# ishine/StyleTTS-ZS

Measured on AMD Instinct MI355X. Metric: synthesized audio-sec/sec (whole job) + p50 utterance latency, 3-s ref -> 5-s target, higher is better.
Workload: dtype bf16; 1 GPU; configs[2]: batch 64/GPU, 5-s targets, 2-step distilled style diffusion, CFG 5; global_batch=64, seq_len=200, parallelism=dp1 (utterance shards), spec=v0, graph=True, branch_streams=False, streams=2, schedule=pipe, stagger=0

## Files before the change

### include/stzs.h

```cpp
#ifndef STZS_H
#define STZS_H

#include <stddef.h>
#include <stdint.h>

#ifdef __cplusplus
extern "C" {
#endif

#define STZS_OK 0
#define STZS_EINVAL (-1)
#define STZS_ESHAPE (-2)
#define STZS_EDTYPE (-3)
#define STZS_EHIP (-4)

enum { STZS_F32 = 0, STZS_BF16 = 1, STZS_I32 = 2, STZS_F8 = 3  };
enum { STZS_ACT_NONE = 0, STZS_ACT_LEAKY = 1, STZS_ACT_SNAKE = 2, STZS_ACT_GELU = 3, STZS_ACT_SILU = 4 };
enum { STZS_PRO_NONE = 0, STZS_PRO_ADAIN = 1 };
#define STZS_CONV_A_DMA 8

int stzs_init(int device);
const char* stzs_strerror(int code);
int stzs_version(void);

// ... 42 lines not shown
#define STZS_CONV_UPS_NOISE 4096
#define STZS_CONV_MRFV_NARROW 8192
#define STZS_CONV_W_FRAG32X3 16384
#define STZS_CONV_MRFV_T128 32768
#define STZS_CONV_RING 65536
#define STZS_CONV_SK_TICKET 131072
size_t stzs_conv_rows_workspace(int64_t rows, int32_t Co, int32_t kgroups);
int stzs_conv1d(const stzs_conv_args* a, void* stream);
int stzs_conv1d_group(const stzs_conv_args* a, int n, void* stream);

typedef struct stzs_stats_args {
    const void* x;
    float* mean;
    float* rstd;
    void* partial;
    int64_t ld, bs, stat_bs;
    int32_t B, T, C, dtype;
    float eps, pad_f;
} stzs_stats_args;
size_t stzs_chan_stats_workspace(int B, int T, int C);
int stzs_chan_stats(const stzs_stats_args* a, void* stream);
int stzs_chan_stats_partial(const stzs_stats_args* a, void* stream);
int stzs_chan_stats_final(const stzs_stats_args* a, int chunk_rows, void* stream);
int stzs_chan_stats_final_group(const stzs_stats_args* a, int n, int chunk_rows, void* stream);

typedef struct stzs_rowln_args {
    const void* x;
    void* y;
    const float* G;
    const float* Bt;
    int64_t ldx, ldy, gs, bs;
    int32_t R, C, gdiv, in_dtype, out_dtype, act;
    float gadd, eps, slope, pad_f;
    float* y_scale;
} stzs_rowln_args;
int stzs_row_layernorm(const stzs_rowln_args* a, void* stream);
int stzs_ln_linear(const stzs_conv_args* a, const stzs_rowln_args* ln, void* stream);

typedef struct stzs_quant_args {
    const void* x;
    void* y;
    float* scale;
    int64_t ldx, ldy;
    int32_t R, C;
} stzs_quant_args;
int stzs_quant_rows(const stzs_quant_args* a, void* stream);
// ... 281 lines not shown
```

### styletts-zs_amd/csrc/norm.hip

```cpp
#include "common.hpp"
#include "rowln.hpp"

namespace {

constexpr int STAT_ROWS = 256;
constexpr int STAT_CG = 32;

template <typename T>
__global__ __launch_bounds__(256) void chan_stats_partial(const stzs_stats_args a, int nchunk) {
    __shared__ float red[8][STAT_CG * 8][2];
    const int tid = threadIdx.x, tx = tid & 31, ty = tid >> 5;
    const int chunk = blockIdx.x, b = blockIdx.y;
    const int cv = blockIdx.z * STAT_CG + tx;
    const int c = cv * 8;
    float s[8], q[8];
#pragma unroll
    for (int j = 0; j < 8; ++j) s[j] = q[j] = 0.f;
    const int r0 = chunk * STAT_ROWS, r1 = min(a.T, r0 + STAT_ROWS);
    const T* X = reinterpret_cast<const T*>(a.x) + (long)b * a.bs;
    if (c < a.C) {
        int r = r0 + ty;
        for (; r + 24 < r1; r += 32) {
            float v[4][8];
#pragma unroll
// ... 62 lines not shown
            s += (double)v.x;
            q += (double)v.y;
        }
    }
    red[g][cl][0] = s;
    red[g][cl][1] = q;
    __syncthreads();
    if (tid < FIN_CH && c < a.C) {
        s = q = 0.0;
#pragma unroll
        for (int y = 0; y < 8; ++y) {
            s += red[y][tid][0];
            q += red[y][tid][1];
        }
        float mu, rs;
        stat_finish(s, q, a.T, a.eps, mu, rs);
        a.mean[(long)b * a.stat_bs + c] = mu;
        a.rstd[(long)b * a.stat_bs + c] = rs;
    }
}

__global__ __launch_bounds__(256) void chan_stats_final(const stzs_stats_args a, int nchunk) {
    stats_final_body(a, nchunk, blockIdx.x, blockIdx.y);
}

struct StatsGroup {
    stzs_stats_args a[3];
    int nchunk[3];
};
__global__ __launch_bounds__(256) void chan_stats_final_group(const StatsGroup g) {
    const int z = blockIdx.z;
    const stzs_stats_args& a = z == 0 ? g.a[0] : (z == 1 ? g.a[1] : g.a[2]);
    if ((int)blockIdx.x >= a.B || (int)blockIdx.y * FIN_CH >= a.C) return;
    stats_final_body(a, z == 0 ? g.nchunk[0] : (z == 1 ? g.nchunk[1] : g.nchunk[2]), blockIdx.x, blockIdx.y);
}


template <typename TI, typename TO>
__global__ __launch_bounds__(256) void row_ln(const stzs_rowln_args a) {
    const long r = (long)blockIdx.x * 4 + (threadIdx.x >> 6);
    if (r >= a.R) return;
    stzs_ln::row_ln_one<TI, TO>(a, r, threadIdx.x & 63);
}

__global__ __launch_bounds__(256) void quant_rows(const stzs_quant_args a) {
    constexpr int MAXV = 4;
// ... 45 lines not shown
    if (rc != STZS_OK) return rc;
    STZS_LAUNCH_CHECK();
    return STZS_OK;
}

extern "C" int stzs_chan_stats(const stzs_stats_args* a, void* stream) {
    if (!a || !a->x || !a->mean || !a->rstd || !a->partial) return STZS_EINVAL;
    hipStream_t s = reinterpret_cast<hipStream_t>(stream);
    int nchunk = 0;
    const int rc = chan_stats_pass1(a, s, &nchunk);
    if (rc != STZS_OK) return rc;
    STZS_LAUNCH_CHECK();
    hipLaunchKernelGGL(chan_stats_final, dim3(a->B, (a->C + FIN_CH - 1) / FIN_CH), dim3(256), 0, s, *a, nchunk);
    STZS_LAUNCH_CHECK();
    return STZS_OK;
}

extern "C" int stzs_chan_stats_final(const stzs_stats_args* a, int chunk_rows, void* stream) {
    if (!a || !a->mean || !a->rstd || !a->partial) return STZS_EINVAL;
    if (a->B <= 0 || a->T <= 0 || a->C <= 0 || chunk_rows <= 0) return STZS_ESHAPE;
    hipStream_t s = reinterpret_cast<hipStream_t>(stream);
    const int nchunk = (a->T + chunk_rows - 1) / chunk_rows;
    hipLaunchKernelGGL(chan_stats_final, dim3(a->B, (a->C + FIN_CH - 1) / FIN_CH), dim3(256), 0, s, *a, nchunk);
    STZS_LAUNCH_CHECK();
    return STZS_OK;
}

extern "C" int stzs_chan_stats_final_group(const stzs_stats_args* a, int n, int chunk_rows, void* stream) {
    if (!a || n < 1 || n > 3 || chunk_rows <= 0) return STZS_EINVAL;
    StatsGroup g = {};
    int gx = 0, gy = 0;
    for (int i = 0; i < n; ++i) {
        if (!a[i].mean || !a[i].rstd || !a[i].partial) return STZS_EINVAL;
        if (a[i].B <= 0 || a[i].T <= 0 || a[i].C <= 0) return STZS_ESHAPE;
        g.a[i] = a[i];
        g.nchunk[i] = (a[i].T + chunk_rows - 1) / chunk_rows;
        gx = a[i].B > gx ? a[i].B : gx;
        const int ny = (a[i].C + FIN_CH - 1) / FIN_CH;
        gy = ny > gy ? ny : gy;
    }
    hipLaunchKernelGGL(chan_stats_final_group, dim3(gx, gy, n), dim3(256), 0, reinterpret_cast<hipStream_t>(stream), g);
    STZS_LAUNCH_CHECK();
    return STZS_OK;
}

extern "C" int stzs_row_layernorm(const stzs_rowln_args* a, void* stream) {
// ... 37 lines not shown
```

### styletts-zs_amd/csrc/ups.hip

```cpp
#include "common.hpp"

namespace {

constexpr int NTH = 256;
#ifndef STZS_UPS_P
#define STZS_UPS_P 288
#endif
constexpr int P = STZS_UPS_P;
constexpr int rows_of(int bt) { return bt + 1; }
constexpr int tile_of(int bt) { return (rows_of(bt) * P + 15) & ~15; }
constexpr int RING = 4;

template <int NCH, bool HR, bool NZ, int BT = 128>
__global__ __launch_bounds__(NTH, NCH * tile_of(BT) <= 80 * 1024 ? 2 : 1) void ups_conv(const stzs_conv_args a, int ctw) {
    extern __shared__ __attribute__((aligned(16))) unsigned char smem[];
    constexpr int ROWS = rows_of(BT), TILE = tile_of(BT);
    constexpr int SB = (ROWS + 15) / 16;
    constexpr int MT = BT / 16;
    constexpr int NK = NCH * 8;
    constexpr int NKW = NK + (NZ ? 1 : 0);
    const int tid = threadIdx.x, lane = tid & 63, wave = tid >> 6;
    const int tpb = (a.T_out + BT - 1) / BT;
    const int nx = gridDim.x;
    const int lin = (a.flags & STZS_CONV_LINEAR_IDS) ? blockIdx.y * nx + blockIdx.x
                                                      : xcd_remap(blockIdx.y * nx + blockIdx.x, nx * gridDim.y);
    const int gy = lin / nx, bx = lin - gy * nx;
    const int bq = bx / tpb;
    const int q0 = (bx - bq * tpb) * BT;
    const int ncol = a.ups * a.Co;
    const int nct = (ncol + 127) / 128;
    const int ct0 = gy * ctw, ct1 = min(nct, ct0 + ctw);
    const int J = (ct1 - ct0) * NK;
    const bf16x8* Wf = reinterpret_cast<const bf16x8*>(a.w) + (long)ct0 * NKW * 512 + wave * 128 + lane;
    bf16x8 wf[RING][2];
// ... 24 lines not shown
#pragma unroll
        for (int i = 0; i < SB; ++i) {
            const int r = rsub + 16 * i;
            const int tin = q0 - 1 + r;
            const bool ok = c_ok && tin >= 0 && tin < a.T_in;
            const uint32_t w[4] = {raw[i].x, raw[i].y, raw[i].z, raw[i].w};
            uint32_t o[4];
#pragma unroll
            for (int p = 0; p < 4; ++p) {
                float y0 = __uint_as_float(w[p] << 16) + 0.f, y1 = __uint_as_float(w[p] & 0xFFFF0000u) + 0.f;
                if (lrelu) {
                    y0 = y0 >= 0.f ? y0 : y0 * slope;
                    y1 = y1 >= 0.f ? y1 : y1 * slope;
                }
                o[p] = ok ? pack2bf(y0, y1) : 0u;
            }
            if (r < ROWS) *reinterpret_cast<uint4*>(smem + cc * TILE + r * P + cv * 16) = make_uint4(o[0], o[1], o[2], o[3]);
        }
    }
    __syncthreads();
    const int g = lane >> 4, n = lane & 15;
    const int xoff0 = (lane & 15) * P + (lane >> 4) * 16;
    const int t_hi = a.T_final + a.refl - 1;
    const bf16_t* Rb = reinterpret_cast<const bf16_t*>(a.res) + (long)bq * a.bsr;
    bf16_t* Y = reinterpret_cast<bf16_t*>(a.y) + (long)bq * a.bsy;
    f32x4 acc[2][MT];
    bf16x8 xf[MT];
    for (int ct = ct0; ct < ct1; ++ct) {
        const int jb = (ct - ct0) * NK;
        const int col0 = ct * 128 + wave * 32 + g * 8;
        const int ph = col0 / a.Co, cof = col0 - ph * a.Co;
        const bool col_ok = col0 < ncol;
        const int cofc = col_ok ? cof : 0;
        uint4 rr[MT];
        int trow[MT];
#pragma unroll
        for (int mt = 0; mt < MT; ++mt) {
            const int q = q0 + mt * 16 + n;
            const int t = q * a.ups + ph - a.ups_pad + a.refl;
            trow[mt] = t;
            const int tc = t < 0 ? 0 : (t > t_hi ? t_hi : t);
            if constexpr (NZ) rr[mt] = *reinterpret_cast<const uint4*>(Rb + (long)tc * a.ldr + g * 8);
            else if constexpr (HR) rr[mt] = *reinterpret_cast<const uint4*>(Rb + (long)tc * a.ldr + cofc);
        }
        bf16x8 wn[2];
        if constexpr (NZ) {
// ... 27 lines not shown
            __builtin_amdgcn_sched_barrier(0);
        }
        if constexpr (NZ) {
#pragma unroll
            for (int mt = 0; mt < MT; ++mt) {
                const bf16x8 hf = __builtin_bit_cast(bf16x8, rr[mt]);
                acc[0][mt] = __builtin_amdgcn_mfma_f32_16x16x32_bf16(wn[0], hf, acc[0][mt], 0, 0, 0);
                acc[1][mt] = __builtin_amdgcn_mfma_f32_16x16x32_bf16(wn[1], hf, acc[1][mt], 0, 0, 0);
            }
        }
        if (a.flags & 4) continue;
        float corr[8] = {0.f, 0.f, 0.f, 0.f, 0.f, 0.f, 0.f, 0.f};
        if constexpr (NZ) {
            if (a.refl && q0 == 0 && n == 0 && trow[0] == 2 && col_ok) {
#pragma unroll 1
                for (int j = 0; j < 32; ++j) {
                    const float d = bf2f(Rb[j]) - bf2f(Rb[2 * a.ldr + j]);
#pragma unroll
                    for (int i = 0; i < 8; ++i) corr[i] = fmaf(a.gate[(long)(cof + i) * 32 + j], d, corr[i]);
                }
            }
        }
#pragma unroll
        for (int mt = 0; mt < MT; ++mt) {
            const int q = q0 + mt * 16 + n;
            const int t = trow[mt];
            const int tp = t - a.refl;
            const bool ok = col_ok && q < a.T_out && tp >= 0 && tp < a.T_final;
            float v[8];
#pragma unroll
            for (int nt = 0; nt < 2; ++nt)
#pragma unroll
                for (int r = 0; r < 4; ++r) v[nt * 4 + r] = acc[nt][mt][r] + bias[nt * 4 + r];
            float w0[8];
#pragma unroll
            for (int i = 0; i < 8; ++i) w0[i] = v[i];
            if constexpr (HR) {
                float f[8];
                unpack8(rr[mt], f);
#pragma unroll
                for (int i = 0; i < 8; ++i) v[i] += f[i];
            }
#pragma unroll
            for (int i = 0; i < 8; ++i) v[i] *= a.alpha;
            if (ok) *reinterpret_cast<uint4*>(Y + (long)t * a.ldy + cof) = pack8(v);
            if (a.refl && ok && t == 2) {
                if constexpr (NZ) {
#pragma unroll
                    for (int i = 0; i < 8; ++i) w0[i] += corr[i];
                } else if constexpr (HR) {
                    float f[8];
                    load8(Rb + cof, f);
#pragma unroll
                    for (int i = 0; i < 8; ++i) w0[i] += f[i];
                }
#pragma unroll
                for (int i = 0; i < 8; ++i) w0[i] *= a.alpha;
                *reinterpret_cast<uint4*>(Y + cof) = pack8(w0);
            }
        }
    }
}

}

__attribute__((visibility("hidden"))) int stzs_ups_conv_launch(const stzs_conv_args& a, hipStream_t s) {
    const bool nz = (a.flags & STZS_CONV_UPS_NOISE) != 0;
    if (nz && (!a.res || !a.gate || a.Co % 128 || a.refl < 0 || a.refl > 1 || a.ldr < 32 || a.ldr % 8 || a.bsr % 8 ||
               (a.refl && a.T_final + a.refl < 3)))
        return STZS_EINVAL;
    if (a.ks != 2 || a.pad != 1 || a.dil != 1 || a.stride != 1 || a.cic != 128 || a.ci_pad % 128 || a.Co % 32 ||
        a.T_out != a.T_in + 1 || a.in_dtype != STZS_BF16 || a.out_dtype != STZS_BF16 || a.pro_mode != STZS_PRO_NONE ||
        (a.pro_act != STZS_ACT_LEAKY && a.pro_act != STZS_ACT_NONE) || a.pro_cscale != 1.f || (a.gate && !nz) || a.acc_in ||
        a.stat_part || a.epi_act != STZS_ACT_NONE || a.ldy % 8 || a.bsy % 8 ||
        (a.res && (a.ldr % 8 || a.bsr % 8 || a.res_tdiv != 1)) || a.co_pad < a.ups * a.Co)
        return STZS_ESHAPE;
    const int nch = a.ci_pad / 128;
    const int nct = (a.ups * a.Co + 127) / 128;
    static const int bt_env = [] {
        const char* e = getenv("STZS_UPS_BT");
        return e ? atoi(e) : 0;
    }();
    const int BT = bt_env == 64 || bt_env == 128 ? bt_env : (nch > 2 ? 64 : 128);
    const int nqt = a.B * ((a.T_out + BT - 1) / BT);
    const int target = 4 * stzs_cu_count();
    int groups = 1;
    while (groups < nct && (long)nqt * groups < target) ++groups;
    const int ctw = (nct + groups - 1) / groups;
    groups = (nct + ctw - 1) / ctw;
    const size_t lds = (size_t)nch * (BT == 64 ? tile_of(64) : tile_of(128));
    void (*k)(stzs_conv_args, int) = nullptr;
    const bool R = a.res != nullptr;
#define STZS_UPS_PICK(N, B_)                                                                                    \
    k = nz ? ups_conv<N, false, true, B_> : R ? ups_conv<N, true, false, B_> : ups_conv<N, false, false, B_>;
    switch (nch * (BT == 64 ? -1 : 1)) {
        case 1: STZS_UPS_PICK(1, 128) break;
        case 2: STZS_UPS_PICK(2, 128) break;
// ... 15 lines not shown
```

### styletts-zs_amd/stzs/_lib.py

```python
from __future__ import annotations

import ctypes as C
import os

_HERE = os.path.dirname(os.path.abspath(__file__))
LIB_PATH = os.environ.get("STZS_LIB", os.path.join(_HERE, "libstzs_hip.so"))

F32, BF16, I32, F8 = 0, 1, 2, 3
OK, EINVAL, ESHAPE, EDTYPE, EHIP = 0, -1, -2, -3, -4
ACT_NONE, ACT_LEAKY, ACT_SNAKE, ACT_GELU, ACT_SILU = 0, 1, 2, 3, 4
PRO_NONE, PRO_ADAIN = 0, 1
CONV_STAT_ROWS = 64
CONV_W_LANE16 = 16
CONV_W_NARROW32 = 32
CONV_W_FRAG32 = 256
CONV_W_F32 = 64
CONV_W_X3 = 1024
CONV_LINEAR_IDS = 128
CONV_ROWS = 2048
CONV_UPS_NOISE = 4096
CONV_MRFV_NARROW = 8192
CONV_MRFV_T128 = 32768
CONV_RING = 65536
CONV_SK_TICKET = 131072
# ... 157 lines not shown
    d = Tensor()
    d.data = t.data_ptr()
    d.dtype = dtype if dtype is not None else {torch.float32: F32, torch.bfloat16: BF16, torch.int32: I32,
                                                torch.float8_e4m3fn: F8, torch.uint8: BF16}[t.dtype]
    d.ndim = t.dim()
    for k in range(t.dim()):
        d.shape[k] = t.shape[k]
        d.stride[k] = t.stride(k)
    return d


def params(ints=(), floats=()) -> Params:
    p = Params()
    for k, v in enumerate(ints):
        p.i[k] = int(v)
    for k, v in enumerate(floats):
        p.f[k] = float(v)
    return p


EXPORTS = ["stzs_init", "stzs_strerror", "stzs_version", "stzs_conv1d", "stzs_conv1d_group", "stzs_conv_splitk_workspace",
           "stzs_conv_rows_workspace",
           "stzs_chan_stats_workspace",
           "stzs_chan_stats", "stzs_chan_stats_partial", "stzs_chan_stats_final", "stzs_chan_stats_final_group", "stzs_row_layernorm", "stzs_ln_linear", "stzs_quant_rows", "stzs_attention", "stzs_lstm_workspace", "stzs_lstm", "stzs_lstm_pair",
           "stzs_lstm_state_reset", "stzs_predictor_prep",
           "stzs_durations", "stzs_alignment", "stzs_gather_rows", "stzs_adain_dwup", "stzs_f0n_down",
           "stzs_harmonic_source", "stzs_istft", "stzs_istft_stream", "stzs_istft_stream_span",
           "stzs_stft_frames", "stzs_log_mel", "stzs_stft_logmel", "stzs_pool_rows", "stzs_code_quantize",
           "stzs_dn_cond", "stzs_dn_cond_steps", "stzs_adaln_expand", "stzs_cfg_euler",
           "stzs_state_init", "stzs_mean_rows", "stzs_copy2d", "stzs_embed", "stzs_embed_f32", "stzs_dn_cond_steps_f32", "stzs_pack_conv_size", "stzs_pack_conv",
           "stzs_pack_lstm", "stzs_pack_lstm_x3"] + [f"stzs_{o}{sfx}" for o in GENERIC_OPS for sfx in ("", "_workspace")]

_lib = None


class StzsError(RuntimeError):
    pass


def load():
    global _lib
    if _lib is not None:
        return _lib
    if not os.path.exists(LIB_PATH):
        raise StzsError(f"libstzs_hip.so not found at {LIB_PATH}: run `python styletts-zs_amd/build.py` "
                        "(the product path has no CPU fallback)")
    L = C.CDLL(LIB_PATH)
    P = C.POINTER
    sig = {
        "stzs_init": ([i32], i32),
        "stzs_strerror": ([i32], C.c_char_p),
        "stzs_version": ([], i32),
        "stzs_conv1d": ([P(ConvArgs), vp], i32),
        "stzs_conv1d_group": ([P(ConvArgs), i32, vp], i32),
        "stzs_conv_splitk_workspace": ([i64, i32, i32], C.c_size_t),
        "stzs_conv_rows_workspace": ([i64, i32, i32], C.c_size_t),
        "stzs_chan_stats_workspace": ([i32, i32, i32], C.c_size_t),
        "stzs_chan_stats": ([P(StatsArgs), vp], i32),
        "stzs_chan_stats_partial": ([P(StatsArgs), vp], i32),
        "stzs_chan_stats_final": ([P(StatsArgs), i32, vp], i32),
        "stzs_chan_stats_final_group": ([P(StatsArgs), i32, i32, vp], i32),
        "stzs_row_layernorm": ([P(RowLNArgs), vp], i32),
        "stzs_ln_linear": ([P(ConvArgs), P(RowLNArgs), vp], i32),
        "stzs_quant_rows": ([P(QuantArgs), vp], i32),
        "stzs_attention": ([P(AttnArgs), vp], i32),
        "stzs_lstm_workspace": ([i32, i32, i32], C.c_size_t),
        "stzs_lstm": ([P(LstmArgs), vp], i32),
        "stzs_lstm_pair": ([P(LstmArgs), P(LstmArgs), vp], i32),
        "stzs_lstm_state_reset": ([vp, vp, vp], i32),
        "stzs_predictor_prep": ([P(PrPrepArgs), vp], i32),
        "stzs_durations": ([P(DurArgs), vp], i32),
        "stzs_alignment": ([P(AlignArgs), vp], i32),
        "stzs_gather_rows": ([P(GatherArgs), vp], i32),
        "stzs_adain_dwup": ([P(DwupArgs), vp], i32),
        "stzs_f0n_down": ([P(F0nArgs), vp], i32),
        "stzs_harmonic_source": ([P(SourceArgs), vp], i32),
        "stzs_istft": ([P(IstftArgs), vp], i32),
        "stzs_istft_stream": ([P(IstftStreamArgs), vp], i32),
        "stzs_istft_stream_span": ([i32, i32, i32, i32, i32, P(i64), P(i64)], i32),
        "stzs_stft_frames": ([P(FramesArgs), vp], i32),
        "stzs_log_mel": ([P(LogMelArgs), vp], i32),
        "stzs_stft_logmel": ([P(StftMelArgs), vp], i32),
        "stzs_pool_rows": ([P(PoolArgs), vp], i32),
# ... 36 lines not shown
```

### styletts-zs_amd/stzs/engine.py

```python
from __future__ import annotations

import ctypes as C
import math
import os
from dataclasses import dataclass
from functools import partial

import numpy as np
import torch

from . import _lib as L
from .spec import Spec
from .weights import ConvW, PackedModel

_DT = {torch.float32: L.F32, torch.bfloat16: L.BF16, torch.float8_e4m3fn: L.F8}
DN_SPLITK = {}
LATENCY_DN_SPLITK = dict(ff2=4)
DN_ROWS = {}
LATENCY_DN_ROWS = dict(inp=1, qkv=1, o=1, q=1, co=1, ff1=1, ff2=4, out=1)
TE_SPLITK = 0
LATENCY_TE_SPLITK = 4
BLK_SPLITK = 0
LATENCY_BLK_SPLITK = 16

# ... 34 lines not shown


def _on(v):
    return v != "0"


_KNOBS = (
    ("dur_overlap", "STZS_DUR_OVERLAP", "1", lambda v: bool(int(v))),
    ("dn_splitk", "STZS_DN_SPLITK", DN_SPLITK, _table),
    ("dn_rows", "STZS_DN_ROWS", DN_ROWS, _table),
    ("te_splitk", "STZS_TE_SPLITK", TE_SPLITK, int),
    ("blk_splitk", "STZS_BLK_SPLITK", BLK_SPLITK, int),
    ("defer_stats", "STZS_DEFER_STATS", lambda eng: "1" if eng.blk_splitk else "0", _on),
    ("mrf_trio", "STZS_MRF_TRIO", "1", _on),
    ("f0n_pair", "STZS_F0N_PAIR", "1", _on),
    ("kv_fuse", "STZS_KV_FUSE", "1", _on),
    ("small_rows", "STZS_SMALL_ROWS", "1", _on),
    ("ln_fuse", "STZS_LN_FUSE", "1", _on),
    ("rows16", "STZS_ROWS16", "1", _on),
    ("rows16_split", "STZS_ROWS16_SPLIT", "1", _on),
    ("rows16_maxk", "STZS_ROWS16_MAXK", "512", int),
    ("ups_noise_fused", "STZS_UPS_NOISE", "1", _on),
    ("noise_super", "STZS_NOISE_SUPER", "1", _on),
    ("mrfx", "STZS_MRFX", "1", _on),
    ("conv_flags", "STZS_CONV_FLAGS", "0", lambda v: int(v, 0)),
)


def _rup(x, m):
    return (x + m - 1) // m * m


@dataclass
class Act:
    t: torch.Tensor
    c0: int = 0
    C: int = -1

    def __post_init__(self):
        if self.C < 0:
            self.C = self.t.shape[-1] - self.c0

    @property
    def B(self):
        return self.t.shape[0]

# ... 28 lines not shown
    if steps == 1:
        return [spec.sigma_max, 0.0]
    if steps == 2:
        return [spec.sigma_max, 0.5, 0.0]
    lo, hi = spec.sigma_min ** (1 / spec.rho), spec.sigma_max ** (1 / spec.rho)
    return [(hi + i / (steps - 1) * (lo - hi)) ** spec.rho for i in range(steps)] + [0.0]


def edm_coeffs(spec: Spec, sigma: float):
    sd = spec.sigma_data
    return dict(c_in=1.0 / math.sqrt(sigma ** 2 + sd ** 2), c_skip=sd ** 2 / (sigma ** 2 + sd ** 2),
                c_out=sigma * sd / math.sqrt(sigma ** 2 + sd ** 2), c_noise=math.log(sigma) / 4.0)


def fourier_features(spec: Spec, c_noise: float) -> np.ndarray:
    half = spec.dn_fourier // 2
    f = np.exp(-math.log(10000.0) * np.arange(half) / half)
    arg = 1000.0 * c_noise * f
    return np.concatenate([np.cos(arg), np.sin(arg)]).astype(np.float32)


class _StatsRef:

    def __init__(self, eng, part, ld, nch, T, B, mean, rstd, chunk_rows):
        self.eng, self.part, self.ld, self.nch, self.T, self.B = eng, part, ld, nch, T, B
        self.mean, self.rstd, self.chunk_rows, self.done = mean, rstd, chunk_rows, False

    def final_args(self, s):
        s.mean, s.rstd, s.partial = self.mean.data_ptr(), self.rstd.data_ptr(), self.part.data_ptr()
        s.stat_bs, s.B, s.T, s.C, s.eps = self.ld, self.B, self.T, self.ld, 1e-5
        return s

    def finalize(self):
        if not self.done:
            self.eng._raw(self.eng.lib.stzs_chan_stats_final, "chan_stats_final",
                          C.byref(self.final_args(L.StatsArgs())), self.chunk_rows)
            self.done = True

    def mean_ptr(self):
        self.finalize()
        return self.mean.data_ptr()

    def rstd_ptr(self):
        self.finalize()
        return self.rstd.data_ptr()


class _StatPtr:

    def __init__(self, ref, which):
        self.ref, self.which = ref, which

    def data_ptr(self):
        return self.ref.mean_ptr() if self.which == 0 else self.ref.rstd_ptr()

    def tensor(self):
        self.ref.finalize()
        return self.ref.mean if self.which == 0 else self.ref.rstd

# ... 134 lines not shown
        if rows > 1 or splitk > 1:
            self._conv_splitk(a, cw, x, splitk, rows, collect, what)
        if pro_ref is not None:
            self._conv_stats_in(a, cw, pro_ref, pre_ln)
        st = self._conv_stats_out(a, cw, y, stats_key, collect) if stats_key is not None else None
        fn, args, fused = self._conv_entry(a, cw, x, res, res_tdiv, gate, pre_ln, st)
        if collect is not None:
            assert len(args) == 1 and pre_ln is None and post_ln is None and attn is None, what
            collect.append(a)
        else:
            if pre_ln is not None and not fused:
                self._call(self.lib.stzs_row_layernorm, pre_ln, what + ".ln", cost=_ln_cost(pre_ln))
            rec = {} if self.timer is None else dict(
                shape=(cw.ks, dil, a.T_out, cw.Co),
                cost=partial(_conv_cost, cw, x, y, a.T_out, res, acc_in, pre_ln if fused else None))
            self._call(fn, a, what, args=args, **rec)
        if post_ln is not None:
            self._call(self.lib.stzs_row_layernorm, post_ln, what + ".ln", cost=_ln_cost(post_ln))
        if attn is not None:
            self.attention(*attn)
        if st is None:
            return y
        slab, Cc, mean, rstd, defer, ntile = st
        ref = _StatsRef(self, slab, Cc, ntile, a.T_out, y.B, mean, rstd, L.CONV_STAT_ROWS)
        if not defer:
            ref.finalize()
            return y, (mean, rstd, Cc)
        return y, (_StatPtr(ref, 0), _StatPtr(ref, 1), Cc)

    def _conv_fill(self, cw, x, y, what, *, T_out, pad, dil, stride, pro, pro_act, pro_slope, pro_alpha, cscale, res,
                   res_tdiv, acc_in, alpha, beta, gate, gate_bs, epi_act, epi_slope, ups_pad, T_final, refl, x_scale):
        a = L.ConvArgs()
        a.x, a.w, a.y = x.ptr, self._t(cw.w).data_ptr(), y.ptr
        a.bias = self._t(cw.b).data_ptr() if cw.b is not None else None
        a.ldx, a.bsx, a.ldy, a.bsy = x.ld, x.bs, y.ld, y.bs
        T = x.T
        a.B, a.T_in, a.Ci, a.Co, a.ks, a.dil, a.stride, a.pad = x.B, T, cw.Ci, cw.Co, cw.ks, dil, stride, pad
        assert x.C == cw.Ci, (what, x.C, cw.Ci)
        if cw.ups:
            a.T_out = T + 1
            a.ups, a.ups_pad, a.T_final, a.refl = cw.ups, ups_pad, T_final, refl
            a.pad = 1
        else:
            a.T_out = T_out if T_out is not None else (T + 2 * pad - dil * (cw.ks - 1) - 1) // stride + 1
        a.ci_pad, a.co_pad, a.cic = cw.ci_pad, cw.co_pad, cw.cic
        a.in_dtype, a.out_dtype = x.dt, y.dt
        pro_ref = None
# ... 82 lines not shown
            splitk = min(splitk, 16, cw.ci_pad // cw.cic)
        if splitk > 1 and (a.flags & 8) and not cw.f8 and cw.wx3 is None and cw.w32 is None:
            nb = self.lib.stzs_conv_splitk_workspace(x.B * x.T, cw.co_pad, splitk)
            assert nb > 0, (what, splitk)
            a.splitk, a.splitk_ws = splitk, self._scratch("sk_ws", nb // 4).data_ptr()
            a.splitk_ctr = self._counters("sk_ctr", nb // (splitk * 32768)).data_ptr()
        elif splitk > 1 and _conv_generic(a.flags, cw):
            tiles = x.B * ((a.T_out + 127) // 128) * (cw.co_pad // 128)
            a.splitk = splitk
            gs = f".g{len(collect)}" if collect is not None else ""
            a.splitk_ws = self._scratch("csk_ws" + gs, tiles * splitk * 16384).data_ptr()
            a.splitk_ctr = self._counters("csk_ctr" + gs, tiles).data_ptr()

    def _conv_stats_in(self, a, cw, pro_ref, pre_ln):
        if _conv_generic(a.flags, cw) and pre_ln is None and pro_ref.nch <= 8:
            a.pro_part, a.pro_ld, a.pro_nch, a.pro_T, a.pro_eps = pro_ref.part.data_ptr(), pro_ref.ld, pro_ref.nch, \
                pro_ref.T, 1e-5
        else:
            a.pro_mean, a.pro_rstd = pro_ref.mean_ptr(), pro_ref.rstd_ptr()

    def _conv_stats_out(self, a, cw, y, stats_key, collect):
        Cc = _rup(cw.Co, 8)
        ntile = (a.T_out + L.CONV_STAT_ROWS - 1) // L.CONV_STAT_ROWS
        defer = collect is not None or (self.defer_stats and ntile <= 8)
        slab = self._scratch("stat_slab." + stats_key, y.B * ntile * Cc * 2, 1024) if defer else \
            self._scratch("stat_slab", y.B * ntile * Cc * 2)
        a.stat_part, a.stat_ld = slab.data_ptr(), Cc
        return (slab, Cc, self.buf(stats_key + ".m", (y.B, Cc), torch.float32),
                self.buf(stats_key + ".r", (y.B, Cc), torch.float32), defer, ntile)

    def _conv_entry(self, a, cw, x, res, res_tdiv, gate, pre_ln, st):
        if not (a.flags & L.CONV_ROWS):
            return self.lib.stzs_conv1d, (C.byref(a),), False
        nk = cw.ci_pad // 32
        if pre_ln is not None:
            fused = a.splitk <= 1 and res is None and gate is None and \
                st is None and pre_ln.C == cw.Ci == cw.ci_pad and nk in (4, 8, 16) and pre_ln.out_dtype == L.BF16 and \
                pre_ln.act == L.ACT_NONE and (pre_ln.x or 0) % 16 == 0 and pre_ln.ldx % 8 == 0 and \
                pre_ln.gdiv > 0 and pre_ln.R < (1 << 22) - 16 and \
                (not pre_ln.G or (pre_ln.gs % 8 == 0 and pre_ln.G % 32 == 0)) and \
                (not pre_ln.Bt or (pre_ln.bs % 8 == 0 and pre_ln.Bt % 32 == 0))
            if fused:
                return self.lib.stzs_ln_linear, (C.byref(a), C.byref(pre_ln)), True
        r16 = (pre_ln is None and self.rows16 and st is None and
               (res is None or res_tdiv == 1) and x.ptr % 16 == 0 and x.ld % 8 == 0 and x.bs % 8 == 0)
        r16_split = r16 and self.rows16_split and a.splitk in (2, 4) and nk % a.splitk == 0 and \
            nk // a.splitk in (4, 8, 16)
# ... 714 lines not shown
            sd = self._consts.get(skey)
            if sd is None:
                host = torch.as_tensor(np.asarray(seeds, dtype=np.uint32).view(np.int32).copy())
                sd = self._consts[skey] = host.to(self.device)
        pref = self.buf("gen.pref", (B, nh, T80), torch.float32)
        dt = self.dec_dt
        hb = self.buf("gen.har", (B, self._har_rows(Tf), _rup(S.har_ch, 32)), dt, zero=True)
        har = Act(hb[:, :Tf], 0, S.har_ch)
        a = L.SourceArgs()
        a.f0, a.seeds, a.merge_w, a.prefix, a.har = F0.data_ptr(), sd.data_ptr(), W.t(W.src_merge).data_ptr(), \
            pref.data_ptr(), har.ptr
        a.ldf, a.ldh, a.bsh = F0.stride(0), har.ld, har.bs
        a.B, a.T80, a.hop, a.n_fft, a.hop_s, a.nh = B, T80, S.hop, S.n_fft, S.istft_hop, nh
        a.sr, a.sine_amp, a.noise_std, a.voiced_thr = float(S.sr), S.sine_amp, S.noise_std, S.voiced_threshold
        a.har_dtype = har.dt
        self._call(self.lib.stzs_harmonic_source, a, "harmonic_source",
                   cost=(0, B * T80 * 4 * (1 + 2 * nh) + B * Tf * S.har_ch * har.t.element_size()))
        return har

    def _har_rows(self, Tf: int) -> int:
        s = math.prod(self.spec.up_rates[1:]) if len(self.spec.up_rates) > 1 else 1
        return _rup(Tf, s)

    def upsample(self, x: Act, har: Act, i: int) -> Act:
        S, W = self.spec, self.W
        B = x.B
        n_up = len(S.up_rates)
        r, k = S.up_rates[i], S.up_kernels[i]
        c = S.gen_ch[i]
        last = i == n_up - 1
        Tcur = x.T
        Tn = Tcur * r + (1 if last else 0)
        dt = self.dec_dt
        xu = self.act(f"gen.x{i}", B, Tn, c, dt)
        nzw = self.W.ups_nz[i] if (self.ups_noise_fused and i < len(self.W.ups_nz)) else None
        if nzw is not None and dt == torch.bfloat16 and har.ld >= 32:
            self.conv(nzw, x, xu, pro_act=L.ACT_LEAKY, pro_slope=0.1, ups_pad=(k - r) // 2, T_final=Tcur * r,
                      refl=1 if last else 0, res=Act(har.t, 0, har.ld), flags=L.CONV_UPS_NOISE,
                      gate=self._t(nzw.nz32).data_ptr(), what=f"ups{i}")
            return xu
        xsrc = self.act(f"gen.xsrc{i}", B, Tn, c, dt)
        sup = W.noise_sup[i] if (not last and i < len(W.noise_sup)) else None
        sf0 = int(np.prod(S.up_rates[i + 1:])) if not last else 1
        rows_alloc = har.bs // har.ld
        if (sup is not None and self.noise_super and har.dt == L.BF16 and har.bs % (sf0 * har.ld) == 0 and
                rows_alloc // sf0 >= Tn + 1 and sf0 * har.ld == sup.Ci and har.t.stride(1) == har.ld):
            hs = har.t.as_strided((B, rows_alloc // sf0, sf0 * har.ld), (har.bs, sf0 * har.ld, 1))
            self.conv(sup, Act(hs), xsrc, pad=1, T_out=Tn, what=f"noise_conv{i}")
        elif not last:
            self.conv(W.noise_conv[i], har.sl(0, S.har_ch), xsrc, stride=sf0, pad=(sf0 + 1) // 2, T_out=Tn,
                      what=f"noise_conv{i}")
        else:
            self.conv(W.noise_conv[i], har.sl(0, S.har_ch), xsrc, T_out=Tn, what=f"noise_conv{i}")
        self.conv(W.ups[i], x, xu, pro_act=L.ACT_LEAKY, pro_slope=0.1, ups_pad=(k - r) // 2, T_final=Tcur * r,
                  refl=1 if last else 0, res=xsrc, what=f"ups{i}")
        return xu

    def conv_post(self, x: Act) -> Act:
        S, W = self.spec, self.W
        post = self.act("gen.post", x.B, x.T, S.har_ch, torch.float32)
        self.conv(W.conv_post, x, Act(post.t, 0, S.har_ch), pad=3, pro_act=L.ACT_LEAKY, pro_slope=0.01,
                  what="conv_post")
        return post

    def istft(self, post: Act) -> torch.Tensor:
        S = self.spec
        B, Tcur = post.B, post.T
        Nout = (Tcur - 1) * S.istft_hop
        wav = self.buf("gen.wav", (B, Nout), torch.float32)
        a = L.IstftArgs()
        a.post, a.wav, a.ldp, a.bsp, a.bsw = post.ptr, wav.data_ptr(), post.ld, post.bs, Nout
        a.B, a.Tf, a.n_fft, a.hop_s = B, Tcur, S.n_fft, S.istft_hop
        self._call(self.lib.stzs_istft, a, "istft", cost=(0, B * Tcur * S.har_ch * 4 + B * Nout * 4))
        return wav

    def generator(self, x: Act, F0: torch.Tensor, seeds, gbd, trace=None, istft=True, har: Act = None):
        S, W = self.spec, self.W
        ng = W.dec_norm
        if har is None:
            har = self.sine_gen(F0, seeds)
        if trace is not None:
            trace["har"] = har
        for i in range(len(S.up_rates)):
            xu = self.upsample(x, har, i)
            if trace is not None:
                trace[f"mrf_in{i}"] = xu
            x = self.mrf(xu, i, gbd, ng)
            if trace is not None:
                trace[f"mrf_out{i}"] = x
        post = self.conv_post(x)
        if trace is not None:
            trace["post"] = post
        if not istft:
            return post
        return self.istft(post)

    def _istft_chunk(self, rows_ptr, ldp, bsp, B, f0, Fc, fin, wav, tails, i):
        S = self.spec
        n0, n1 = C.c_int64(), C.c_int64()
        halo = self.lib.stzs_istft_stream_span(f0, Fc, fin, S.n_fft, S.istft_hop, C.byref(n0), C.byref(n1))
        L.check(min(halo, 0), "istft_stream_span")
        assert halo <= 8
        a = L.IstftStreamArgs()
        a.post = rows_ptr
        a.tail_in = tails[i % 2].data_ptr() if f0 > 0 else None
        a.tail_out = tails[(i + 1) % 2].data_ptr() if not fin else None
        a.wav = wav.data_ptr() + n0.value * 4
        a.ldp, a.bsp, a.bsw, a.ldt = ldp, bsp, wav.shape[1], tails[0].shape[2]
        a.B, a.f0, a.Fc, a.final_chunk, a.n_fft, a.hop_s = B, f0, Fc, fin, S.n_fft, S.istft_hop
        self._call(self.lib.stzs_istft_stream, a, "istft_stream")
# ... 101 lines not shown
        self.launches += rc

    def _finalize_group(self, refs):
        arr = (L.StatsArgs * len(refs))()
        for s, r in zip(arr, refs):
            r.final_args(s)
        assert len({r.chunk_rows for r in refs}) == 1
        self._raw(self.lib.stzs_chan_stats_final_group, "chan_stats_final_group", arr, len(refs), refs[0].chunk_rows)
        for r in refs:
            r.done = True

    def _rb_c1(self, lw, x: Act, y: Act, st, gbd, ng, stats_key, collect=None):
        k, dil = lw["k"], lw["dil"]
        o1, c1 = ng.offsets[lw["n1"]]
        return self.conv(lw["c1"], x, y, pad=dil * (k - 1) // 2, dil=dil,
                         pro=(*st, gbd.data_ptr() + o1 * 4, ng.total, c1), pro_act=L.ACT_SNAKE, pro_alpha=lw["a1"],
                         stats_key=stats_key, collect=collect, what="rb.c1")[1]

    def _rb_c2(self, lw, x: Act, y: Act, st, res: Act, gbd, ng, **kw):
        o2, c2 = ng.offsets[lw["n2"]]
        return self.conv(lw["c2"], x, y, pad=(lw["k"] - 1) // 2, pro=(*st, gbd.data_ptr() + o2 * 4, ng.total, c2),
                         pro_act=L.ACT_SNAKE, pro_alpha=lw["a2"], res=res, what="rb.c2", **kw)

    def _mrf_trio(self, x: Act, i, gbd, ng):
        S, W = self.spec, self.W
        B, T, c = x.B, x.T, x.C
        dt = x.t.dtype
        nk = len(S.rb_kernels)
        xs = self.act(f"gen.xs{i}", B, T, c, dt)
        t1 = [self.act(f"gen.t1_{i}.{j}", B, T, c, dt) for j in range(nk)]
        bufs = [(self.act(f"gen.ba{i}.{j}", B, T, c, dt), self.act(f"gen.bb{i}.{j}", B, T, c, dt)) for j in range(nk)]
        mx, rx, sb = self.stats(x, f"gen.sx{i}")
        cur, cm, cr = [x] * nk, [mx] * nk, [rx] * nk
        nl = len(W.rb[i][0])
        for m in range(nl):
            grp = []
            st1 = [self._rb_c1(res[m], cur[j], t1[j], (cm[j], cr[j], sb), gbd, ng, f"gen.st{i}.{j}", collect=grp)
                   for j, res in enumerate(W.rb[i])]
            self._launch_group(grp, "rb.c1")
            self._finalize_group([st[0].ref for st in st1])
            if m == nl - 1:
                for j, res in enumerate(W.rb[i]):
                    self._rb_c2(res[m], t1[j], xs, (*st1[j][:2], sb), cur[j], gbd, ng, alpha=1.0 / nk,
                                acc_in=(xs if j > 0 else None), beta=1.0)
                break
            grp = []
            outs = [bufs[j][0] if cur[j] is not bufs[j][0] else bufs[j][1] for j in range(nk)]
            st2 = [self._rb_c2(res[m], t1[j], outs[j], (*st1[j][:2], sb), cur[j], gbd, ng,
                               stats_key=f"gen.sc{i}.{j}.{m % 2}", collect=grp)[1] for j, res in enumerate(W.rb[i])]
            self._launch_group(grp, "rb.c2")
            self._finalize_group([st[0].ref for st in st2])
            for j in range(nk):
                cur[j], (cm[j], cr[j], _) = outs[j], st2[j]
        return xs

    def _mrf_trio_on(self, x: Act, i) -> bool:
        rb = self.W.rb[i]
        return (self.mrf_trio and self.timer is None and x.B <= 4 and tuple(self.spec.rb_kernels) == (3, 7, 11) and
                len({len(res) for res in rb}) == 1 and all(r["k"] == k for res, k in zip(rb, (3, 7, 11)) for r in res))

    def mrf(self, x: Act, i, gbd, ng):
        S, W = self.spec, self.W
        if self._mrf_trio_on(x, i):
            return self._mrf_trio(x, i, gbd, ng)
        B, T, c = x.B, x.T, x.C
        dt = x.t.dtype
        xs = self.act(f"gen.xs{i}", B, T, c, dt)
        bufA = self.act(f"gen.ba{i}", B, T, c, dt)
        bufB = self.act(f"gen.bb{i}", B, T, c, dt)
        t1 = self.act(f"gen.t1_{i}", B, T, c, dt)
        mx, rx, sb = self.stats(x, f"gen.sx{i}")
        nk = len(S.rb_kernels)
        for j, res in enumerate(W.rb[i]):
            cur, cm, cr = x, mx, rx
            for m, lw in enumerate(res):
                tm, tr, _ = self._rb_c1(lw, cur, t1, (cm, cr, sb), gbd, ng, f"gen.st{i}")
                last = m == len(res) - 1
                out = xs if last else (bufA if cur is not bufA else bufB)
                r2 = self._rb_c2(lw, t1, out, (tm, tr, sb), cur, gbd, ng, alpha=(1.0 / nk) if last else 1.0,
                                 acc_in=(xs if (last and j > 0) else None), beta=1.0,
                                 stats_key=None if last else f"gen.sc{i}.{m % 2}")
                if not last:
                    _, (cm, cr, _) = r2
                    cur = out
        return xs

    def twin(self) -> "StyleTTSZS":
        t = object.__new__(StyleTTSZS)
        t.__dict__.update(self.__dict__)
        t._bufs, t._retired, t._consts, t._side, t._branch, t.launches, t.timer = {}, [], {}, {}, "", 0, None
        t._depth = 0
        t.status = torch.zeros(1, dtype=torch.int32, device=self.device)
        return t

# ... 93 lines not shown
```

Before: 19660 audio-s/s.

## Fuse MRF input channel statistics into upsample conv epilogue

The upsample transposed-conv kernel now accumulates per-channel sum and sum-of-squares of its bf16 outputs. It reduces them across 16 lanes with DPP moves and writes per-slot partials, and a new slot-based finalize kernel turns those partials into mean/rstd. MRF then reuses these statistics instead of running a separate chan_stats pass over the upsampled activation. This saves a full read of the large upsampled tensor per stage, at the cost of extra epilogue work and partial-slab writes in the ups kernel, plus a separate finalize launch.

```diff
diff --git a/include/stzs.h b/include/stzs.h
--- a/include/stzs.h
+++ b/include/stzs.h
@@ -88,6 +88,7 @@
 int stzs_chan_stats(const stzs_stats_args* a, void* stream);
 int stzs_chan_stats_partial(const stzs_stats_args* a, void* stream);
 int stzs_chan_stats_final(const stzs_stats_args* a, int chunk_rows, void* stream);
+int stzs_chan_stats_final_slots(const stzs_stats_args* a, int nslot, void* stream);
 int stzs_chan_stats_final_group(const stzs_stats_args* a, int n, int chunk_rows, void* stream);
 
 typedef struct stzs_rowln_args {
diff --git a/styletts-zs_amd/csrc/norm.hip b/styletts-zs_amd/csrc/norm.hip
--- a/styletts-zs_amd/csrc/norm.hip
+++ b/styletts-zs_amd/csrc/norm.hip
@@ -108,6 +108,44 @@
 
 __global__ __launch_bounds__(256) void chan_stats_final(const stzs_stats_args a, int nchunk) {
     stats_final_body(a, nchunk, blockIdx.x, blockIdx.y);
+}
+
+__global__ __launch_bounds__(256) void chan_stats_final_slots(const stzs_stats_args a, int nslot) {
+    __shared__ double red[8][FIN_CH][2];
+    const int tid = threadIdx.x, cl = tid & (FIN_CH - 1), g = tid >> 5;
+    const int b = blockIdx.x, c = blockIdx.y * FIN_CH + cl;
+    double s = 0.0, q = 0.0;
+    if (c < a.C) {
+        const float2* P = reinterpret_cast<const float2*>(a.partial) + (long)b * nslot * a.C + c;
+        for (int k = g; k < nslot; k += 128) {
+            float2 v[16];
+#pragma unroll
+            for (int u = 0; u < 16; ++u) {
+                const int ku = k + 8 * u;
+                v[u] = ku < nslot ? P[(long)ku * a.C] : make_float2(0.f, 0.f);
+            }
+#pragma unroll
+            for (int u = 0; u < 16; ++u) {
+                s += (double)v[u].x;
+                q += (double)v[u].y;
+            }
+        }
+    }
+    red[g][cl][0] = s;
+    red[g][cl][1] = q;
+    __syncthreads();
+    if (tid < FIN_CH && c < a.C) {
+        s = q = 0.0;
+#pragma unroll
+        for (int y = 0; y < 8; ++y) {
+            s += red[y][tid][0];
+            q += red[y][tid][1];
+        }
+        float mu, rs;
+        stat_finish(s, q, a.T, a.eps, mu, rs);
+        a.mean[(long)b * a.stat_bs + c] = mu;
+        a.rstd[(long)b * a.stat_bs + c] = rs;
+    }
 }
 
 struct StatsGroup {
@@ -199,6 +237,15 @@
     hipStream_t s = reinterpret_cast<hipStream_t>(stream);
     const int nchunk = (a->T + chunk_rows - 1) / chunk_rows;
     hipLaunchKernelGGL(chan_stats_final, dim3(a->B, (a->C + FIN_CH - 1) / FIN_CH), dim3(256), 0, s, *a, nchunk);
+    STZS_LAUNCH_CHECK();
+    return STZS_OK;
+}
+
+extern "C" int stzs_chan_stats_final_slots(const stzs_stats_args* a, int nslot, void* stream) {
+    if (!a || !a->mean || !a->rstd || !a->partial) return STZS_EINVAL;
+    if (a->B <= 0 || a->T <= 0 || a->C <= 0 || nslot <= 0) return STZS_ESHAPE;
+    hipStream_t s = reinterpret_cast<hipStream_t>(stream);
+    hipLaunchKernelGGL(chan_stats_final_slots, dim3(a->B, (a->C + FIN_CH - 1) / FIN_CH), dim3(256), 0, s, *a, nslot);
     STZS_LAUNCH_CHECK();
     return STZS_OK;
 }
diff --git a/styletts-zs_amd/csrc/ups.hip b/styletts-zs_amd/csrc/ups.hip
--- a/styletts-zs_amd/csrc/ups.hip
+++ b/styletts-zs_amd/csrc/ups.hip
@@ -10,6 +10,21 @@
 constexpr int rows_of(int bt) { return bt + 1; }
 constexpr int tile_of(int bt) { return (rows_of(bt) * P + 15) & ~15; }
 constexpr int RING = 4;
+
+STZS_DEV void row_sum16_n8(float* x) {
+#pragma unroll
+    for (int step = 0; step < 4; ++step) {
+#pragma unroll
+        for (int i = 0; i < 8; ++i) {
+            const int xi = __float_as_int(x[i]);
+            const int y = step == 0   ? __builtin_amdgcn_mov_dpp(xi, 0xB1, 0xF, 0xF, true)
+                          : step == 1 ? __builtin_amdgcn_mov_dpp(xi, 0x4E, 0xF, 0xF, true)
+                          : step == 2 ? __builtin_amdgcn_mov_dpp(xi, 0x141, 0xF, 0xF, true)
+                                      : __builtin_amdgcn_mov_dpp(xi, 0x140, 0xF, 0xF, true);
+            x[i] += __int_as_float(y);
+        }
+    }
+}
 
 template <int NCH, bool HR, bool NZ, int BT = 128>
 __global__ __launch_bounds__(NTH, NCH * tile_of(BT) <= 80 * 1024 ? 2 : 1) void ups_conv(const stzs_conv_args a, int ctw) {
@@ -80,6 +95,9 @@
     const int g = lane >> 4, n = lane & 15;
     const int xoff0 = (lane & 15) * P + (lane >> 4) * 16;
     const int t_hi = a.T_final + a.refl - 1;
+    const bool stat = a.stat_part != nullptr;
+    const int nslot = ((a.T_out + 63) >> 6) * a.ups + a.refl;
+    float* SP = reinterpret_cast<float*>(a.stat_part) + (long)bq * nslot * a.stat_ld * 2;
     const bf16_t* Rb = reinterpret_cast<const bf16_t*>(a.res) + (long)bq * a.bsr;
     bf16_t* Y = reinterpret_cast<bf16_t*>(a.y) + (long)bq * a.bsy;
     f32x4 acc[2][MT];
@@ -153,41 +171,82 @@
             }
         }
 #pragma unroll
-        for (int mt = 0; mt < MT; ++mt) {
-            const int q = q0 + mt * 16 + n;
-            const int t = trow[mt];
-            const int tp = t - a.refl;
-            const bool ok = col_ok && q < a.T_out && tp >= 0 && tp < a.T_final;
-            float v[8];
-#pragma unroll
-            for (int nt = 0; nt < 2; ++nt)
-#pragma unroll
-                for (int r = 0; r < 4; ++r) v[nt * 4 + r] = acc[nt][mt][r] + bias[nt * 4 + r];
-            float w0[8];
-#pragma unroll
-            for (int i = 0; i < 8; ++i) w0[i] = v[i];
-            if constexpr (HR) {
-                float f[8];
-                unpack8(rr[mt], f);
-#pragma unroll
-                for (int i = 0; i < 8; ++i) v[i] += f[i];
-            }
-#pragma unroll
-            for (int i = 0; i < 8; ++i) v[i] *= a.alpha;
-            if (ok) *reinterpret_cast<uint4*>(Y + (long)t * a.ldy + cof) = pack8(v);
-            if (a.refl && ok && t == 2) {
-                if constexpr (NZ) {
-#pragma unroll
-                    for (int i = 0; i < 8; ++i) w0[i] += corr[i];
-                } else if constexpr (HR) {
+        for (int h = 0; h < MT / 4; ++h) {
+            float ss[8], sq[8];
+#pragma unroll
+            for (int i = 0; i < 8; ++i) ss[i] = sq[i] = 0.f;
+#pragma unroll
+            for (int m = 0; m < 4; ++m) {
+                const int mt = h * 4 + m;
+                const int q = q0 + mt * 16 + n;
+                const int t = trow[mt];
+                const int tp = t - a.refl;
+                const bool ok = col_ok && q < a.T_out && tp >= 0 && tp < a.T_final;
+                float v[8];
+#pragma unroll
+                for (int nt = 0; nt < 2; ++nt)
+#pragma unroll
+                    for (int r = 0; r < 4; ++r) v[nt * 4 + r] = acc[nt][mt][r] + bias[nt * 4 + r];
+                float w0[8];
+#pragma unroll
+                for (int i = 0; i < 8; ++i) w0[i] = v[i];
+                if constexpr (HR) {
                     float f[8];
-                    load8(Rb + cof, f);
-#pragma unroll
-                    for (int i = 0; i < 8; ++i) w0[i] += f[i];
-                }
-#pragma unroll
-                for (int i = 0; i < 8; ++i) w0[i] *= a.alpha;
-                *reinterpret_cast<uint4*>(Y + cof) = pack8(w0);
+                    unpack8(rr[mt], f);
+#pragma unroll
+                    for (int i = 0; i < 8; ++i) v[i] += f[i];
+                }
+#pragma unroll
+                for (int i = 0; i < 8; ++i) v[i] *= a.alpha;
+                const uint4 o = pack8(v);
+                if (ok) *reinterpret_cast<uint4*>(Y + (long)t * a.ldy + cof) = o;
+                if (stat && ok) {
+                    float f[8];
+                    unpack8(o, f);
+#pragma unroll
+                    for (int i = 0; i < 8; ++i) {
+                        ss[i] += f[i];
+                        sq[i] = fmaf(f[i], f[i], sq[i]);
+                    }
+                }
+                if (a.refl && ok && t == 2) {
+                    if constexpr (NZ) {
+#pragma unroll
+                        for (int i = 0; i < 8; ++i) w0[i] += corr[i];
+                    } else if constexpr (HR) {
+                        float f[8];
+                        load8(Rb + cof, f);
+#pragma unroll
+                        for (int i = 0; i < 8; ++i) w0[i] += f[i];
+                    }
+#pragma unroll
+                    for (int i = 0; i < 8; ++i) w0[i] *= a.alpha;
+                    const uint4 o0 = pack8(w0);
+                    *reinterpret_cast<uint4*>(Y + cof) = o0;
+                    if (stat) {
+                        float f[8];
+                        unpack8(o0, f);
+                        float* Pr = SP + ((long)(nslot - 1) * a.stat_ld + cof) * 2;
+#pragma unroll
+                        for (int i = 0; i < 8; ++i) {
+                            Pr[2 * i] = f[i];
+                            Pr[2 * i + 1] = f[i] * f[i];
+                        }
+                    }
+                }
+            }
+            if (stat) {
+                row_sum16_n8(ss);
+                row_sum16_n8(sq);
+                const int qh = q0 + h * 64;
+                if (n == 0 && col_ok && qh < a.T_out) {
+                    float* Pp = SP + ((long)((qh >> 6) * a.ups + ph) * a.stat_ld + cof) * 2;
+#pragma unroll
+                    for (int i = 0; i < 8; ++i) {
+                        Pp[2 * i] = ss[i];
+                        Pp[2 * i + 1] = sq[i];
+                    }
+                }
             }
         }
     }
@@ -203,7 +262,7 @@
     if (a.ks != 2 || a.pad != 1 || a.dil != 1 || a.stride != 1 || a.cic != 128 || a.ci_pad % 128 || a.Co % 32 ||
         a.T_out != a.T_in + 1 || a.in_dtype != STZS_BF16 || a.out_dtype != STZS_BF16 || a.pro_mode != STZS_PRO_NONE ||
         (a.pro_act != STZS_ACT_LEAKY && a.pro_act != STZS_ACT_NONE) || a.pro_cscale != 1.f || (a.gate && !nz) || a.acc_in ||
-        a.stat_part || a.epi_act != STZS_ACT_NONE || a.ldy % 8 || a.bsy % 8 ||
+        (a.stat_part && (a.stat_ld < a.Co || (a.refl && a.T_final < 2))) || a.epi_act != STZS_ACT_NONE || a.ldy % 8 || a.bsy % 8 ||
         (a.res && (a.ldr % 8 || a.bsr % 8 || a.res_tdiv != 1)) || a.co_pad < a.ups * a.Co)
         return STZS_ESHAPE;
     const int nch = a.ci_pad / 128;
diff --git a/styletts-zs_amd/stzs/_lib.py b/styletts-zs_amd/stzs/_lib.py
--- a/styletts-zs_amd/stzs/_lib.py
+++ b/styletts-zs_amd/stzs/_lib.py
@@ -203,7 +203,7 @@
 EXPORTS = ["stzs_init", "stzs_strerror", "stzs_version", "stzs_conv1d", "stzs_conv1d_group", "stzs_conv_splitk_workspace",
            "stzs_conv_rows_workspace",
            "stzs_chan_stats_workspace",
-           "stzs_chan_stats", "stzs_chan_stats_partial", "stzs_chan_stats_final", "stzs_chan_stats_final_group", "stzs_row_layernorm", "stzs_ln_linear", "stzs_quant_rows", "stzs_attention", "stzs_lstm_workspace", "stzs_lstm", "stzs_lstm_pair",
+           "stzs_chan_stats", "stzs_chan_stats_partial", "stzs_chan_stats_final", "stzs_chan_stats_final_slots", "stzs_chan_stats_final_group", "stzs_row_layernorm", "stzs_ln_linear", "stzs_quant_rows", "stzs_attention", "stzs_lstm_workspace", "stzs_lstm", "stzs_lstm_pair",
            "stzs_lstm_state_reset", "stzs_predictor_prep",
            "stzs_durations", "stzs_alignment", "stzs_gather_rows", "stzs_adain_dwup", "stzs_f0n_down",
            "stzs_harmonic_source", "stzs_istft", "stzs_istft_stream", "stzs_istft_stream_span",
@@ -240,6 +240,7 @@
         "stzs_chan_stats": ([P(StatsArgs), vp], i32),
         "stzs_chan_stats_partial": ([P(StatsArgs), vp], i32),
         "stzs_chan_stats_final": ([P(StatsArgs), i32, vp], i32),
+        "stzs_chan_stats_final_slots": ([P(StatsArgs), i32, vp], i32),
         "stzs_chan_stats_final_group": ([P(StatsArgs), i32, i32, vp], i32),
         "stzs_row_layernorm": ([P(RowLNArgs), vp], i32),
         "stzs_ln_linear": ([P(ConvArgs), P(RowLNArgs), vp], i32),
diff --git a/styletts-zs_amd/stzs/engine.py b/styletts-zs_amd/stzs/engine.py
--- a/styletts-zs_amd/stzs/engine.py
+++ b/styletts-zs_amd/stzs/engine.py
@@ -80,6 +80,7 @@
     ("rows16_maxk", "STZS_ROWS16_MAXK", "512", int),
     ("ups_noise_fused", "STZS_UPS_NOISE", "1", _on),
     ("noise_super", "STZS_NOISE_SUPER", "1", _on),
+    ("ups_stats", "STZS_UPS_STATS", "1", _on),
     ("mrfx", "STZS_MRFX", "1", _on),
     ("conv_flags", "STZS_CONV_FLAGS", "0", lambda v: int(v, 0)),
 )
@@ -154,9 +155,9 @@
 
 class _StatsRef:
 
-    def __init__(self, eng, part, ld, nch, T, B, mean, rstd, chunk_rows):
+    def __init__(self, eng, part, ld, nch, T, B, mean, rstd, chunk_rows, slots=False):
         self.eng, self.part, self.ld, self.nch, self.T, self.B = eng, part, ld, nch, T, B
-        self.mean, self.rstd, self.chunk_rows, self.done = mean, rstd, chunk_rows, False
+        self.mean, self.rstd, self.chunk_rows, self.done, self.slots = mean, rstd, chunk_rows, False, slots
 
     def final_args(self, s):
         s.mean, s.rstd, s.partial = self.mean.data_ptr(), self.rstd.data_ptr(), self.part.data_ptr()
@@ -165,8 +166,12 @@
 
     def finalize(self):
         if not self.done:
-            self.eng._raw(self.eng.lib.stzs_chan_stats_final, "chan_stats_final",
-                          C.byref(self.final_args(L.StatsArgs())), self.chunk_rows)
+            if self.slots:
+                self.eng._raw(self.eng.lib.stzs_chan_stats_final_slots, "chan_stats_final",
+                              C.byref(self.final_args(L.StatsArgs())), self.nch)
+            else:
+                self.eng._raw(self.eng.lib.stzs_chan_stats_final, "chan_stats_final",
+                              C.byref(self.final_args(L.StatsArgs())), self.chunk_rows)
             self.done = True
 
     def mean_ptr(self):
@@ -347,7 +352,8 @@
         if st is None:
             return y
         slab, Cc, mean, rstd, defer, ntile = st
-        ref = _StatsRef(self, slab, Cc, ntile, a.T_out, y.B, mean, rstd, L.CONV_STAT_ROWS)
+        ref = _StatsRef(self, slab, Cc, ntile, a.T_final + a.refl, y.B, mean, rstd, L.CONV_STAT_ROWS, slots=True) \
+            if cw.ups else _StatsRef(self, slab, Cc, ntile, a.T_out, y.B, mean, rstd, L.CONV_STAT_ROWS)
         if not defer:
             ref.finalize()
             return y, (mean, rstd, Cc)
@@ -476,7 +482,10 @@
     def _conv_stats_out(self, a, cw, y, stats_key, collect):
         Cc = _rup(cw.Co, 8)
         ntile = (a.T_out + L.CONV_STAT_ROWS - 1) // L.CONV_STAT_ROWS
-        defer = collect is not None or (self.defer_stats and ntile <= 8)
+        if cw.ups:
+            assert collect is None
+            ntile = ntile * cw.ups + a.refl
+        defer = collect is not None or (self.defer_stats and ntile <= 8 and not cw.ups)
         slab = self._scratch("stat_slab." + stats_key, y.B * ntile * Cc * 2, 1024) if defer else \
             self._scratch("stat_slab", y.B * ntile * Cc * 2)
         a.stat_part, a.stat_ld = slab.data_ptr(), Cc
@@ -1237,7 +1246,7 @@
         s = math.prod(self.spec.up_rates[1:]) if len(self.spec.up_rates) > 1 else 1
         return _rup(Tf, s)
 
-    def upsample(self, x: Act, har: Act, i: int) -> Act:
+    def upsample(self, x: Act, har: Act, i: int, stats=False):
         S, W = self.spec, self.W
         B = x.B
         n_up = len(S.up_rates)
@@ -1249,11 +1258,20 @@
         dt = self.dec_dt
         xu = self.act(f"gen.x{i}", B, Tn, c, dt)
         nzw = self.W.ups_nz[i] if (self.ups_noise_fused and i < len(self.W.ups_nz)) else None
+
+        def skey(cw):
+            return f"gen.sx{i}" if (stats and self.ups_stats and dt == torch.bfloat16 and x.t.dtype == torch.bfloat16 and
+                                    getattr(cw, "frag32", False) and cw.wx3 is None and cw.w32 is None) else None
+
+        def out(r):
+            if not stats:
+                return xu
+            return r if isinstance(r, tuple) else (xu, None)
+
         if nzw is not None and dt == torch.bfloat16 and har.ld >= 32:
-            self.conv(nzw, x, xu, pro_act=L.ACT_LEAKY, pro_slope=0.1, ups_pad=(k - r) // 2, T_final=Tcur * r,
-                      refl=1 if last else 0, res=Act(har.t, 0, har.ld), flags=L.CONV_UPS_NOISE,
-                      gate=self._t(nzw.nz32).data_ptr(), what=f"ups{i}")
-            return xu
+            return out(self.conv(nzw, x, xu, pro_act=L.ACT_LEAKY, pro_slope=0.1, ups_pad=(k - r) // 2, T_final=Tcur * r,
+                                 refl=1 if last else 0, res=Act(har.t, 0, har.ld), flags=L.CONV_UPS_NOISE,
+                                 gate=self._t(nzw.nz32).data_ptr(), stats_key=skey(nzw), what=f"ups{i}"))
         xsrc = self.act(f"gen.xsrc{i}", B, Tn, c, dt)
         sup = W.noise_sup[i] if (not last and i < len(W.noise_sup)) else None
         sf0 = int(np.prod(S.up_rates[i + 1:])) if not last else 1
@@ -1267,9 +1285,9 @@
                       what=f"noise_conv{i}")
         else:
             self.conv(W.noise_conv[i], har.sl(0, S.har_ch), xsrc, T_out=Tn, what=f"noise_conv{i}")
-        self.conv(W.ups[i], x, xu, pro_act=L.ACT_LEAKY, pro_slope=0.1, ups_pad=(k - r) // 2, T_final=Tcur * r,
-                  refl=1 if last else 0, res=xsrc, what=f"ups{i}")
-        return xu
+        return out(self.conv(W.ups[i], x, xu, pro_act=L.ACT_LEAKY, pro_slope=0.1, ups_pad=(k - r) // 2,
+                             T_final=Tcur * r, refl=1 if last else 0, res=xsrc, stats_key=skey(W.ups[i]),
+                             what=f"ups{i}"))
 
     def conv_post(self, x: Act) -> Act:
         S, W = self.spec, self.W
@@ -1297,10 +1315,10 @@
         if trace is not None:
             trace["har"] = har
         for i in range(len(S.up_rates)):
-            xu = self.upsample(x, har, i)
+            xu, st = self.upsample(x, har, i, stats=True)
             if trace is not None:
                 trace[f"mrf_in{i}"] = xu
-            x = self.mrf(xu, i, gbd, ng)
+            x = self.mrf(xu, i, gbd, ng, st=st)
             if trace is not None:
                 trace[f"mrf_out{i}"] = x
         post = self.conv_post(x)
@@ -1448,7 +1466,7 @@
         return self.conv(lw["c2"], x, y, pad=(lw["k"] - 1) // 2, pro=(*st, gbd.data_ptr() + o2 * 4, ng.total, c2),
                          pro_act=L.ACT_SNAKE, pro_alpha=lw["a2"], res=res, what="rb.c2", **kw)
 
-    def _mrf_trio(self, x: Act, i, gbd, ng):
+    def _mrf_trio(self, x: Act, i, gbd, ng, st=None):
         S, W = self.spec, self.W
         B, T, c = x.B, x.T, x.C
         dt = x.t.dtype
@@ -1456,7 +1474,7 @@
         xs = self.act(f"gen.xs{i}", B, T, c, dt)
         t1 = [self.act(f"gen.t1_{i}.{j}", B, T, c, dt) for j in range(nk)]
         bufs = [(self.act(f"gen.ba{i}.{j}", B, T, c, dt), self.act(f"gen.bb{i}.{j}", B, T, c, dt)) for j in range(nk)]
-        mx, rx, sb = self.stats(x, f"gen.sx{i}")
+        mx, rx, sb = st if st is not None else self.stats(x, f"gen.sx{i}")
         cur, cm, cr = [x] * nk, [mx] * nk, [rx] * nk
         nl = len(W.rb[i][0])
         for m in range(nl):
@@ -1485,17 +1503,17 @@
         return (self.mrf_trio and self.timer is None and x.B <= 4 and tuple(self.spec.rb_kernels) == (3, 7, 11) and
                 len({len(res) for res in rb}) == 1 and all(r["k"] == k for res, k in zip(rb, (3, 7, 11)) for r in res))
 
-    def mrf(self, x: Act, i, gbd, ng):
+    def mrf(self, x: Act, i, gbd, ng, st=None):
         S, W = self.spec, self.W
         if self._mrf_trio_on(x, i):
-            return self._mrf_trio(x, i, gbd, ng)
+            return self._mrf_trio(x, i, gbd, ng, st)
         B, T, c = x.B, x.T, x.C
         dt = x.t.dtype
         xs = self.act(f"gen.xs{i}", B, T, c, dt)
         bufA = self.act(f"gen.ba{i}", B, T, c, dt)
         bufB = self.act(f"gen.bb{i}", B, T, c, dt)
         t1 = self.act(f"gen.t1_{i}", B, T, c, dt)
-        mx, rx, sb = self.stats(x, f"gen.sx{i}")
+        mx, rx, sb = st if st is not None else self.stats(x, f"gen.sx{i}")
         nk = len(S.rb_kernels)
         for j, res in enumerate(W.rb[i]):
             cur, cm, cr = x, mx, rx
```

Measured after the change: 19650 audio-s/s. About the same (-0.0%).
